# libAudioFlux/audioFlux

Hardware: AMD Instinct MI355X
Metric: audio frames/sec (mel+MFCC, n_fft=2048 hop=512) (higher is better)
Workload: dtype f32

## Files before the change

audioflux_amd/csrc/hip/afx_melfused2.hip:

```cpp
#include <hip/hip_runtime.h>

#include <cmath>
#include <cstdlib>
#include <cstring>

#include "afx_melplan.h"
#include "afx_melparts.h"
#include "afx_ccblock.h"

#ifdef AFX_V2_NTIN
#define AFX_V2_LOAD(p) __builtin_nontemporal_load(p)
#define AFX_V2_NT true
#else
#define AFX_V2_LOAD(p) (*(p))
#define AFX_V2_NT false
#endif
#ifndef AFX_V2_CCEVERY
#define AFX_V2_CCEVERY 16
#endif
#ifdef AFX_V2_STAMPS
#include <cstdio>
#include <vector>
#endif

namespace {

constexpr int NFFT = 2048;
constexpr int MC = 1024;
constexpr int WAVES = 12;
constexpr int WAVES_CPLX = 12;
__host__ __device__ constexpr int waves_of(bool cplx) { return cplx ? WAVES_CPLX : WAVES; }
constexpr int P1 = 72;
constexpr int PROW_OFF = 5120;
constexpr int PROW_F = 1104;
constexpr int WAVE_LDS = PROW_OFF + PROW_F * 4;
constexpr int CLAIM_LDS = 16;
static_assert(16 * P1 * 8 <= PROW_OFF + 1025 * 4, "exchange image must end before the zero pad");
constexpr int T_WIN = 0;
constexpr int T_TW1 = 8192;
constexpr int T_TW2 = 16384;
constexpr int TW2_PITCH = 144;
constexpr int T_TW3 = 16960;
constexpr int T_BAND = 21056;
__host__ __device__ constexpr int wpitch(int ta, int tb, int pc = 0) { return ta + tb + pc + 4; }
__host__ __device__ constexpr int tab_bytes(int ta, int tb, int pc = 0) { return T_BAND + 64 * wpitch(ta, tb, pc) * 4; }
constexpr int DCT_PITCH = 36;
__host__ __device__ constexpr int block_lds_bytes(int ta, int tb, bool cc, int pc = 0) {
    return tab_bytes(ta, tb, pc) + (cc ? 64 * DCT_PITCH * 4 : 0) + WAVES * WAVE_LDS + CLAIM_LDS;
}

__host__ __device__ constexpr int claim_length(int left, int waves, int minRun) {
    const int g = left / (2 * waves);
    if (left >= 16 * waves) return g >= 16 ? g & ~15 : 16;
    return (g & ~3) > minRun ? g & ~3 : minRun;
}

struct KArgs2 {
    const float *x;
    long long clipStride;
    long long totalFrames;
    int timeLength, hop;
    long long framesPerWg;
    int aligned;
    const float4 *tab;
    const int *meta;
    int specMap, postPow;
    float normValue;
    float *out;
    float *outIm;
    int num;
    const float *dct;
    int ccNum, ccCbrt;
    float *cc;
    float *energy, *rms, *zcr;
    const float *win;
    int binLo, binCount;
    long long outPitch;
    int vecOut;
#ifdef AFX_V2_STAMPS
    unsigned long long *stamps;
#endif
};
#ifdef AFX_V2_STAMPS
constexpr int STAMP_WORDS = 64, STAMP_HEAD = 8;
#endif


#ifndef AFX_PRIO_MASK
#define AFX_PRIO_MASK 0x1E
#endif
#ifndef AFX_PRIO_LEVEL
#define AFX_PRIO_LEVEL 1
#endif
#define MEL_PHASE(p)                                                                                       \
    do {                                                                                                   \
        if (AFX_PRIO_MASK != 0) __builtin_amdgcn_s_setprio(((AFX_PRIO_MASK >> (p)) & 1) ? AFX_PRIO_LEVEL : 0); \
    } while (0)

__device__ __forceinline__ float wave_sum(float v) {
#pragma unroll
    for (int o = 32; o > 0; o >>= 1) v += __shfl_xor(v, o, 64);
    return v;
}

template <int TA, int TB, int SHIFT, bool SPLIT, int CC, bool TEMPORAL, bool CPLX = false, bool STFT = false, int PC = 0>
__global__ __launch_bounds__(waves_of(CPLX) * 64, 3) void k_stft_mel_v2(KArgs2 a) {
    constexpr int NWV = waves_of(CPLX);
    static_assert(!(CPLX && (CC || TEMPORAL)), "complex results: the bank only");
    static_assert(!STFT || (TA == 0 && TB == 0 && !SPLIT && CC == 0 && !TEMPORAL && !CPLX), "STFT instantiations: real rows, no bank");
    static_assert(PC == 0 || (!SPLIT && !STFT), "packed plans hold whole rows");
    extern __shared__ __attribute__((aligned(16))) unsigned char smem[];
    const int lane = threadIdx.x & 63;
    const int wave = threadIdx.x >> 6;
    constexpr int WP = wpitch(TA, TB, PC);
    constexpr int TABB = tab_bytes(TA, TB, PC);
    constexpr int DCTB = CC == 1 ? 64 * DCT_PITCH * 4 : 0;
    unsigned char *wreg = smem + TABB + DCTB + wave * WAVE_LDS;
    float *prow = reinterpret_cast<float *>(wreg + PROW_OFF);

    {
        float4 *s4 = reinterpret_cast<float4 *>(smem);
        for (int i = threadIdx.x + (STFT ? T_TW1 / 16 : 0); i < TABB / 16; i += NWV * 64) s4[i] = a.tab[i];
        if constexpr (STFT) {
            v2 *tw = reinterpret_cast<v2 *>(smem + T_WIN);
            const v2 *w2 = reinterpret_cast<const v2 *>(a.win);
            for (int at = threadIdx.x; at < 1024; at += NWV * 64) {
                const int n1 = 2 * (at >> 7) + (at & 1), l = (at & 127) >> 1;
                tw[at] = w2[64 * n1 + l];
            }
        }
        if constexpr (CC == 1) {
            float *tabD = reinterpret_cast<float *>(smem + TABB);
            for (int i = threadIdx.x; i < 64 * 32; i += NWV * 64) {
                const int l = i >> 5, e = i & 31;
                const int fi = l & 15, g = l >> 4;
                tabD[l * DCT_PITCH + e] =
                    fi < a.ccNum ? a.dct[(long long)fi * a.num + 16 * (e >> 2) + 4 * g + (e & 3)] : 0.f;
            }
        }
        for (int i = 1025 + lane; i < PROW_F; i += 64) prow[i] = 0.f;
        if (threadIdx.x == 0) *reinterpret_cast<int *>(smem + TABB + DCTB + NWV * WAVE_LDS) = 0;
    }
    __syncthreads();

    const int k1 = lane >> 2, m2 = lane & 3;
    const unsigned T0 = lds_addr(smem), W0 = lds_addr(wreg);
    const unsigned aWin = T0 + T_WIN + 16 * lane;
    const unsigned aTw2 = T0 + T_TW2 + TW2_PITCH * m2;
    const unsigned aE1w = W0 + 8 * (8 * (k1 >> 1) + 2 * m2 + (k1 & 1));
    const unsigned aE1r = W0 + 576 * k1 + 16 * m2;
    const unsigned aE2w = W0 + 32 * k1 + 16 * ((m2 >> 1) ^ ((k1 >> 3) & 1)) + 8 * (m2 & 1);
    const int b3l = (lane >> 3) & 1;
    const unsigned aAlo = W0 + 32 * lane + 16 * b3l, aAhi = W0 + 32 * lane + 16 * (1 - b3l);
    const int qm0 = lane == 0 ? 128 : 256 - lane, qm1 = 192 - lane;
    const unsigned aB0lo = W0 + 32 * qm0 + 16 * ((qm0 >> 3) & 1), aB0hi = W0 + 32 * qm0 + 16 * (1 - ((qm0 >> 3) & 1));
    const unsigned aB1lo = W0 + 32 * qm1 + 16 * ((qm1 >> 3) & 1), aB1hi = W0 + 32 * qm1 + 16 * (1 - ((qm1 >> 3) & 1));
    const unsigned aT3lo = T0 + T_TW3 + 32 * lane + 16 * b3l, aT3hi = T0 + T_TW3 + 32 * lane + 16 * (1 - b3l);
    const unsigned R = W0 + PROW_OFF;
    const unsigned aP01 = R + 4 * lane;
    const unsigned aP23 = R + 4 * (lane == 0 ? 128 : lane + 512);
    const unsigned aQs1 = R + 4 * (192 - lane);
    const unsigned aQ23 = R + 4 * (lane == 0 ? 640 : 256 - lane);
    const bool lane0 = (lane == 0);

    constexpr int MROW = PC ? 192 : 128;
    const int startA = STFT ? 0 : a.meta[lane], startB = STFT ? 0 : a.meta[64 + lane], startC = PC ? a.meta[128 + lane] : 0;
    const int rowA = STFT ? -1 : a.meta[MROW + lane], rowB = STFT ? -1 : a.meta[MROW + 64 + lane], rowC = PC ? a.meta[MROW + 128 + lane] : -1;
    const unsigned seg0 = SPLIT ? (unsigned)a.meta[256 + lane] : 0u, seg1 = SPLIT ? (unsigned)a.meta[320 + lane] : 0u;
    const bool contB = PC ? a.meta[384 + lane] != 0 : false, contC = PC ? a.meta[448 + lane] != 0 : false;
    const unsigned apa = R + 4 * startA, apb = R + 4 * startB, apc = R + 4 * startC;
    const unsigned awr = T0 + T_BAND + 4 * WP * lane;
    const unsigned vRaw = 8u * (unsigned)lane, vLane = 4u * (unsigned)lane;
    const bool okA = rowA >= 0, okB = rowB >= 0, okC = rowC >= 0;
    const unsigned vRowA = okA ? 4u * (unsigned)rowA : 0u, vRowB = okB ? 4u * (unsigned)rowB : 0u, vRowC = okC ? 4u * (unsigned)rowC : 0u;
    const long long rowPitch = STFT ? a.outPitch : (long long)a.num;

    const long long wgBeg = (long long)blockIdx.x * a.framesPerWg;
    const int wgN = (int)(a.totalFrames - wgBeg < a.framesPerWg ? a.totalFrames - wgBeg : a.framesPerWg);
    const int minRun = wgN >= 4 * NWV ? 4 : wgN > NWV ? (wgN + NWV - 1) / NWV : 1;
    int *claimed = reinterpret_cast<int *>(smem + TABB + DCTB + NWV * WAVE_LDS);
    const int wgClip = (int)(wgBeg / a.timeLength);
    const unsigned wgT = (unsigned)(wgBeg - (long long)wgClip * a.timeLength);
    auto locate = [&](long long fr, int &c, int &tt) {
        const unsigned at = wgT + (unsigned)(fr - wgBeg);
        c = wgClip + (int)(at / (unsigned)a.timeLength);
        tt = (int)(at % (unsigned)a.timeLength);
    };
    auto claim = [&](long long &rb, long long &re) -> bool {
        int s = wgN, l = 0;
        if (lane0) {
            const int left = wgN - __atomic_load_n(claimed, __ATOMIC_RELAXED);
            if (left > 0) {
                l = claim_length(left, NWV, minRun);
                s = __atomic_fetch_add(claimed, l, __ATOMIC_RELAXED);
            }
        }
        s = __builtin_amdgcn_readfirstlane(s);
        l = __builtin_amdgcn_readfirstlane(l);
        if (s >= wgN) return false;
        rb = wgBeg + s;
        re = wgBeg + (s + l < wgN ? s + l : wgN);
        return true;
    };
    int ccN = 0;
#ifdef AFX_V2_STAMPS
    unsigned long long *stamp = a.stamps + ((long long)blockIdx.x * NWV + wave) * STAMP_WORDS;
    int stampN = 0;
    if (lane0) {
        stamp[0] = __builtin_amdgcn_s_memtime();
        stamp[2] = (unsigned long long)blockIdx.x | ((unsigned long long)wave << 32);
        stamp[4] = (unsigned)__builtin_amdgcn_s_getreg(4 | (0 << 6) | (31 << 11));
        stamp[5] = (unsigned)__builtin_amdgcn_s_getreg(20 | (0 << 6) | (31 << 11));
    }
#endif

    v2 raw[16];
    auto fetch = [&](const float *px, int first) {
        if (a.aligned) {
            const v2 *p2 = reinterpret_cast<const v2 *>(px);
#pragma unroll
            for (int n1 = 0; n1 < 16; ++n1)
                if (n1 >= first) raw[n1] = AFX_V2_LOAD(&p2[64 * n1 + lane]);
        } else {
#pragma unroll
            for (int n1 = 0; n1 < 16; ++n1)
                if (n1 >= first) {
                    const int n = 64 * n1 + lane;
                    raw[n1] = v2{px[2 * n], px[2 * n + 1]};
                }
        }
    };

    auto raw_landed = [&]() {
        if constexpr (SHIFT > 0) {
            VM_WAIT_ALL();
#pragma unroll
            for (int n1 = 0; n1 < 16; ++n1) PIN(raw[n1]);
        }
    };

    auto cc_block = [&](long long fb, long long fbS, int cnt) {
        if constexpr (CC == 2) {
            ccb_rows<SPLIT ? 2 : 4>(a.out, a.cc, a.dct, a.num, a.ccNum, a.ccCbrt, fb, cnt, lane);
        } else {
        VM_WAIT_ALL();
        int ln = lane;
        PIN(ln);
        const int fi = ln & 15, g = ln >> 4;
        fbS = uniform64(fbS);
        const float *const srows = a.out + fbS * 128;
        const unsigned vsrc = 512u * (unsigned)(fi < cnt ? fi : cnt - 1) + 16u * (unsigned)g;
        const unsigned ad = T0 + TABB + 4 * DCT_PITCH * ln;
        v4f acc[4] = {{0.f, 0.f, 0.f, 0.f}, {0.f, 0.f, 0.f, 0.f}, {0.f, 0.f, 0.f, 0.f}, {0.f, 0.f, 0.f, 0.f}};
        constexpr float LOG10_2 = 0.30102999566398120f;
#pragma unroll
        for (int h = 0; h < 2; ++h) {
            v4f av[4], dv[4];
            GLD128X4_L2_S(av[0], av[1], av[2], av[3], vsrc, srows, 256 * h, 256 * h + 64, 256 * h + 128, 256 * h + 192);
#pragma unroll
            for (int u = 0; u < 4; ++u) RD128(dv[u], ad, 16 * (4 * h + u));
            VM_LGKM_WAIT_ALL();
#pragma unroll
            for (int u = 0; u < 4; ++u) PIN(av[u]);
#pragma unroll
            for (int u = 0; u < 4; ++u) PIN(dv[u]);
#pragma unroll
            for (int u = 0; u < 4; ++u) {
                const v4f fl = max4_floor(av[u]);
#pragma unroll
                for (int c = 0; c < 4; ++c) {
                    const float lg = __log2f(fl[c]) * LOG10_2;
                    acc[c] = __builtin_amdgcn_mfma_f32_16x16x4f32(lg, dv[u][c], acc[c], 0, 0, 0);
                }
            }
        }
        const v4f sum = (acc[0] + acc[1]) + (acc[2] + acc[3]);
        if (fi < a.ccNum) {
            const unsigned vcc = 4u * (unsigned)(4 * g * a.ccNum + fi);
            float *const scc = a.cc + fbS * a.ccNum;
#pragma unroll
            for (int reg = 0; reg < 4; ++reg) {
                const int rr = 4 * g + reg;
                if (rr < cnt) GST32_S(vcc, sum[reg], scc + reg * a.ccNum);
            }
        }
        }
        ccN -= cnt;
    };

    long long fClaim, fEndClaim;
    while (claim(fClaim, fEndClaim)) {
    int laneZero = 0;
    PIN(laneZero);
    long long f = fClaim + laneZero;
    const long long fEnd = fEndClaim;
    int clip, t;
    locate(fClaim, clip, t);
    fetch(a.x + (long long)clip * a.clipStride + (long long)t * a.hop, 0);
    long long rowOff = fClaim * rowPitch;
    for (; f < fEnd; ++f) {
        v2 v[16];
        MEL_PHASE(0);
        {
            v4f wv[8];
#pragma unroll
            for (int j = 0; j < 8; ++j) RD128_S(2, wv[j], aWin, T_WIN + 1024 * j);
            LDS_WAIT_N(4);
#pragma unroll
            for (int j = 0; j < 4; ++j) {
                PIN(wv[j]);
                v[2 * j] = raw[2 * j] * lo2(wv[j]);
                v[2 * j + 1] = raw[2 * j + 1] * hi2(wv[j]);
            }
            LDS_WAIT_N(0);
#pragma unroll
            for (int j = 4; j < 8; ++j) {
                PIN(wv[j]);
                v[2 * j] = raw[2 * j] * lo2(wv[j]);
                v[2 * j + 1] = raw[2 * j + 1] * hi2(wv[j]);
            }
        }
        if constexpr (TEMPORAL) {
            float e = 0.f, z = 0.f;
            float prevTop = 0.f;
#pragma unroll
            for (int n1 = 0; n1 < 16; ++n1) {
                e = fmaf(v[n1].x, v[n1].x, e);
                e = fmaf(v[n1].y, v[n1].y, e);
                float py = __shfl_up(v[n1].y, 1, 64);
                if (lane0) py = prevTop;
                const bool first = (n1 == 0) && lane0;
                if (!first && v[n1].x * py < 0.f) z += 1.f;
                if (v[n1].y * v[n1].x < 0.f) z += 1.f;
                prevTop = __shfl(v[n1].y, 63, 64);
            }
            e = wave_sum(e);
            z = wave_sum(z);
            if (lane0) {
                a.energy[f] = e;
                a.rms[f] = sqrtf(e / (float)NFFT);
                a.zcr[f] = (float)((double)z / (double)NFFT);
            }
        }

        MEL_PHASE(1);
        dft16(v);
        {
            v4f tq[8];
#pragma unroll
            for (int j = 0; j < 8; ++j) RD128_S(2, tq[j], aWin, T_TW1 + 1024 * j);
            LDS_WAIT_N(0);
#pragma unroll
            for (int j = 0; j < 8; ++j) PIN(tq[j]);
            v2 o[16];
            o[0] = v[0];
#pragma unroll
            for (int k = 1; k < 16; ++k) o[k] = cmul(v[rev4(k)], (k & 1) ? hi2(tq[k >> 1]) : lo2(tq[k >> 1]));
#pragma unroll
            for (int g = 0; g < 4; ++g) {
                const unsigned b = aE1w + 2304 * g;
                WR2_64_S(0, b, o[4 * g], o[4 * g + 1], 0, 72);
                WR2_64_S(0, b, o[4 * g + 2], o[4 * g + 3], 144, 216);
            }
        }
        if (f + 1 < fEnd) {
            int tn = t + 1, cn = clip;
            if (tn == a.timeLength) {
                tn = 0;
                ++cn;
            }
            const float *pn = a.x + (long long)cn * a.clipStride + (long long)tn * a.hop;
            bool whole = true;
            if constexpr (SHIFT > 0) {
                if (tn != 0) {
                    shift_rows_inplace<SHIFT>(raw);
                    if (a.aligned) {
                        rows_fetch_new_s<SHIFT, AFX_V2_NT>(raw, vRaw, pn + 128 * (16 - SHIFT));
                    } else {
                        int z = 0;
                        VM_WAIT_ALL_AT(z);
                        fetch(pn + z, 16 - SHIFT);
                    }
                    whole = false;
                }
            }
            if (whole) {
                int z = 0;
                if constexpr (SHIFT > 0) VM_WAIT_ALL_AT(z);
                fetch(pn + z, 0);
            }
        }
        wave_lds_sync();
        MEL_PHASE(2);
        {
            v4f rq[8];
#pragma unroll
            for (int jj = 0; jj < 8; ++jj) RD128_S(1, rq[jj], aE1r, 64 * jj);
            wave_lds_sync();
#pragma unroll
            for (int jj = 0; jj < 8; ++jj) {
                PIN(rq[jj]);
                v[2 * jj] = lo2(rq[jj]);
                v[2 * jj + 1] = hi2(rq[jj]);
            }
        }

        MEL_PHASE(3);
        if (!KO_ON(5)) dft16(v);
        {
            v4f tq[8];
#pragma unroll
            for (int j = 0; j < 8; ++j) RD128_S(2, tq[j], aTw2, 16 * j);
            LDS_WAIT_N(0);
#pragma unroll
            for (int j = 0; j < 8; ++j) PIN(tq[j]);
            v2 o[16];
            o[0] = v[0];
#pragma unroll
            for (int j1 = 1; j1 < 16; ++j1) o[j1] = KO_ON(5) ? v[rev4(j1)] : cmul(v[rev4(j1)], (j1 & 1) ? hi2(tq[j1 >> 1]) : lo2(tq[j1 >> 1]));
#pragma unroll
            for (int g = 0; g < 4; ++g) {
                const unsigned b = aE2w + 2048 * g;
                WR2_64_S(0, b, o[4 * g], o[4 * g + 1], 0, 64);
                WR2_64_S(0, b, o[4 * g + 2], o[4 * g + 3], 128, 192);
            }
        }
        wave_lds_sync();

        MEL_PHASE(4);
        float pk[2][4], pq[2][4], p512;
        float ik[CPLX ? 2 : 1][4], iq[CPLX ? 2 : 1][4], i512 = 0.f;
        {
            v4f zalo[2], zahi[2], zblo[2], zbhi[2], wlo[2], whi[2];
            RD128_S(1, zalo[0], aAlo, 0);
            RD128_S(1, zahi[0], aAhi, 0);
            RD128_S(1, zblo[0], aB0lo, 0);
            RD128_S(1, zbhi[0], aB0hi, 0);
            RD128_S(2, wlo[0], aT3lo, 0);
            RD128_S(2, whi[0], aT3hi, 0);
            RD128_S(1, zalo[1], aAlo, 2048);
            RD128_S(1, zahi[1], aAhi, 2048);
            RD128_S(1, zblo[1], aB1lo, 0);
            RD128_S(1, zbhi[1], aB1hi, 0);
            RD128_S(2, wlo[1], aT3lo, 2048);
            RD128_S(2, whi[1], aT3hi, 2048);
#pragma unroll
            for (int s = 0; s < 2; ++s) {
                if (s == 0) LDS_WAIT_N(6);
                else LDS_WAIT_N(0);
                PIN(zalo[s]); PIN(zahi[s]); PIN(zblo[s]); PIN(zbhi[s]); PIN(wlo[s]); PIN(whi[s]);
                v2 za0 = lo2(zalo[s]), za1 = hi2(zalo[s]), za2 = lo2(zahi[s]), za3 = hi2(zahi[s]);
                v2 zb0 = lo2(zblo[s]), zb1 = hi2(zblo[s]), zb2 = lo2(zbhi[s]), zb3 = hi2(zbhi[s]);
                dft4(za0, za1, za2, za3);
                dft4(zb0, zb1, zb2, zb3);
                v2 A0 = za0, A1 = za1, A2 = za2, A3 = za3;
                v2 B0 = zb3, B1 = zb2, B2 = zb1, B3 = zb0;
                if (s == 0) {
                    if constexpr (CPLX) cplx_map(v2{za2.x, -za2.y}, a.specMap == 4, p512, i512);
                    else p512 = za2.x * za2.x + za2.y * za2.y;
                    A2 = lane0 ? zb0 : za2;
                    A3 = lane0 ? zb1 : za3;
                    B0 = lane0 ? za0 : zb3;
                    B1 = lane0 ? za3 : zb2;
                    B2 = lane0 ? zb3 : zb1;
                    B3 = lane0 ? zb2 : zb0;
                }
                if constexpr (CPLX) {
                    const bool sq = a.specMap == 4;
                    const v2 AA[4] = {A0, A1, A2, A3}, BB[4] = {B0, B1, B2, B3};
                    const v2 ww[4] = {lo2(wlo[s]), hi2(wlo[s]), lo2(whi[s]), hi2(whi[s])};
#pragma unroll
                    for (int j = 0; j < 4; ++j) {
                        v2 x, y;
                        split_pair_c(AA[j], BB[j], ww[j], x, y);
                        cplx_map(x, sq, pk[s][j], ik[CPLX ? s : 0][j]);
                        cplx_map(v2{y.x, -y.y}, sq, pq[s][j], iq[CPLX ? s : 0][j]);
                    }
                } else {
                    split_pair(A0, B0, lo2(wlo[s]), pk[s][0], pq[s][0]);
                    split_pair(A1, B1, hi2(wlo[s]), pk[s][1], pq[s][1]);
                    split_pair(A2, B2, lo2(whi[s]), pk[s][2], pq[s][2]);
                    split_pair(A3, B3, hi2(whi[s]), pk[s][3], pq[s][3]);
                }
            }
        }
        if constexpr (CPLX) {
            WR2ST_32(aP01 - PROW_OFF, ik[0][0], ik[0][1], 0, 4);
            WR2ST_32(aP23 - PROW_OFF, ik[0][2], ik[0][3], 0, 4);
            WR2ST_32(aP01 - PROW_OFF, ik[1][0], ik[1][1], 1, 5);
            WR2ST_32(aP01 - PROW_OFF, ik[1][2], ik[1][3], 9, 13);
            WR2ST_32(aQs1 - PROW_OFF, iq[0][1], iq[0][0], 9, 13);
            WR2ST_32(aQ23 - PROW_OFF, iq[0][3], iq[0][2], 0, 4);
            WR2ST_32(aQs1 - PROW_OFF, iq[1][3], iq[1][2], 0, 4);
            WR2ST_32(aQs1 - PROW_OFF, iq[1][1], iq[1][0], 8, 12);
            float *prowI = reinterpret_cast<float *>(wreg);
            if (lane0) prowI[512] = i512;
            prowI[1025 + lane] = 0.f;
            if (lane < PROW_F - 1025 - 64) prowI[1025 + 64 + lane] = 0.f;
        }
        WR2ST_32_S(4, aP01, pk[0][0], pk[0][1], 0, 4);
        WR2ST_32_S(4, aP23, pk[0][2], pk[0][3], 0, 4);
        WR2ST_32_S(4, aP01, pk[1][0], pk[1][1], 1, 5);
        WR2ST_32_S(4, aP01, pk[1][2], pk[1][3], 9, 13);
        WR2ST_32_S(4, aQs1, pq[0][1], pq[0][0], 9, 13);
        WR2ST_32_S(4, aQ23, pq[0][3], pq[0][2], 0, 4);
        WR2ST_32_S(4, aQs1, pq[1][3], pq[1][2], 0, 4);
        WR2ST_32_S(4, aQs1, pq[1][1], pq[1][0], 8, 12);
        if (lane0) prow[512] = p512;
        wave_lds_sync();
#pragma unroll
        for (int pass = 0; pass < (CPLX ? 2 : 1); ++pass) {
        const unsigned bpa = (CPLX && pass) ? apa - PROW_OFF : apa, bpb = (CPLX && pass) ? apb - PROW_OFF : apb;
        const unsigned bpc = (CPLX && pass) ? apc - PROW_OFF : apc;
        if (!CPLX && a.specMap) {
            for (int k = lane; k < 1025; k += 64) {
                const float p = prow[k];
                prow[k] = a.specMap == 1 ? sqrtf(p) : powf(p, a.normValue);
            }
            wave_lds_sync();
        }

        if constexpr (STFT) {
            MEL_PHASE(6);
            raw_landed();
            float *orow = a.out + rowOff;
            if (a.vecOut) {
                const float4 *p4 = reinterpret_cast<const float4 *>(prow);
                float4 *o4 = reinterpret_cast<float4 *>(orow);
                float4 q[4];
#pragma unroll
                for (int i = 0; i < 4; ++i) q[i] = p4[lane + 64 * i];
#pragma unroll
                for (int i = 0; i < 4; ++i) o4[lane + 64 * i] = q[i];
                if (lane0) o4[256] = p4[256];
            } else {
                for (int k = lane; k < a.binCount; k += 64) orow[k] = prow[a.binLo + k];
            }
        } else {
        MEL_PHASE(5);
        float accA, accB, accC = 0.f;
        if constexpr (PC > 0) {
            v2 sA, sB, sC;
            band_stage3<TA, TB, PC, 4, CPLX>(awr, bpa, bpb, bpc, contB, contC, sA, sB, sC);
            accA = sA.x + sA.y;
            accB = sB.x + sB.y;
            accC = sC.x + sC.y;
        } else {
            v2 sA, sB;
            band_stage<TA, TB, 4, CPLX>(awr, bpa, bpb, sA, sB);
            accA = sA.x + sA.y;
            accB = sB.x + sB.y;
        }
        if (!CPLX && !SPLIT && a.postPow) {
            accA = powf(accA, a.normValue);
            accB = powf(accB, a.normValue);
            if constexpr (PC > 0) accC = powf(accC, a.normValue);
        }
        MEL_PHASE(6);
        if (pass == 0) raw_landed();
        if constexpr (CC != 0 && !SPLIT) {
            if (ccN == AFX_V2_CCEVERY) cc_block(f - AFX_V2_CCEVERY, (rowOff >> 7) - AFX_V2_CCEVERY, AFX_V2_CCEVERY);
        }
        float *const srow = ((CPLX && pass) ? a.outIm : a.out) + rowOff;
        if constexpr (SPLIT) {
            float *part = reinterpret_cast<float *>(wreg + (CPLX ? PROW_F * 4 : 0));
            static_assert(PROW_F * 4 + 129 * 4 <= PROW_OFF, "segment sums must fit between the two rows");
            part[lane] = accA;
            part[64 + lane] = accB;
            if (lane0) part[128] = 0.f;
            wave_lds_sync();
#pragma unroll
            for (int h = 0; h < 2; ++h) {
                const unsigned u = h ? seg1 : seg0;
                float sum = part[u & 255u] + part[(u >> 8) & 255u];
                sum += part[(u >> 16) & 255u];
                sum += part[u >> 24];
                if (!CPLX && a.postPow) sum = powf(sum, a.normValue);
                if (lane + 64 * h < a.num) GST32_S(vLane, sum, srow + 64 * h);
            }
        } else {
            if (okA) GST32_S(vRowA, accA, srow);
            if (okB) GST32_S(vRowB, accB, srow);
            if constexpr (PC > 0) {
                if (okC) GST32_S(vRowC, accC, srow);
            }
        }
        if constexpr (CC != 0) {
            ++ccN;
            if (f + 1 == fEnd || (SPLIT && ccN == 16)) cc_block(f + 1 - ccN, (rowOff >> 7) + 1 - ccN, ccN);
        }
        }
        wave_lds_sync();

        }

#ifdef AFX_V2_STAMPS
        ++stampN;
        if (lane0 && (stampN & 15) == 0 && STAMP_HEAD + (stampN >> 4) <= STAMP_WORDS) stamp[STAMP_HEAD - 1 + (stampN >> 4)] = __builtin_amdgcn_s_memtime();
#endif
        rowOff += rowPitch;
        if (++t == a.timeLength) {
            t = 0;
            ++clip;
        }
    }
    }
#ifdef AFX_V2_STAMPS
    if (lane0) {
        stamp[1] = __builtin_amdgcn_s_memtime();
        stamp[3] = (unsigned long long)stampN;
    }
#endif
}

void fill_tables(float *tab, const float *hWindow) {
    const double PI = 3.14159265358979323846;
    float *win = tab + T_WIN / 4, *tw1 = tab + T_TW1 / 4, *tw2 = tab + T_TW2 / 4, *tw3 = tab + T_TW3 / 4;
    for (int n1 = 0; n1 < 16; ++n1)
        for (int l = 0; l < 64; ++l) {
            const int at = 2 * (128 * (n1 >> 1) + 2 * l + (n1 & 1));
            const int n = 64 * n1 + l;
            if (hWindow) {
                win[at] = hWindow[2 * n];
                win[at + 1] = hWindow[2 * n + 1];
            }
            const double ang = -2.0 * PI * (double)(n1 * l) / MC;
            tw1[at] = (float)cos(ang);
            tw1[at + 1] = (float)sin(ang);
        }
    for (int m = 0; m < 4; ++m)
        for (int j = 0; j < 16; ++j) {
            const double ang = -2.0 * PI * (double)(m * j) / 64.0;
            tw2[(TW2_PITCH / 4) * m + 2 * j] = (float)cos(ang);
            tw2[(TW2_PITCH / 4) * m + 2 * j + 1] = (float)sin(ang);
        }
    for (int s = 0; s < 2; ++s)
        for (int l = 0; l < 64; ++l)
            for (int m = 0; m < 4; ++m) {
                int bin = l + 64 * s + 256 * m;
                if (s == 0 && l == 0 && m >= 2) bin = m == 2 ? 128 : 384;
                const double ang = -2.0 * PI * (double)bin / NFFT;
                const int at = 2 * (4 * (64 * s + l) + 2 * ((m >> 1) ^ ((l >> 3) & 1)) + (m & 1));
                tw3[at] = (float)(0.5 * cos(ang));
                tw3[at + 1] = (float)(0.5 * sin(ang));
            }
}

constexpr AfxMelVariant kVariants[] = {{48, 16}, {72, 32}};

long long wg_ranges(long long total, int waves, long long *framesPerWg) {
    const char *e = getenv("AFX_MEL_CUS");
    const int asked = e ? atoi(e) : 0;
    const int cus = asked > 0 ? asked : afx_cu_count();
    long long fpw;
    long long blocks = afx_frame_split(total, cus, waves, 1, &fpw);
    *framesPerWg = fpw * waves;
    if (*framesPerWg > (1ll << 30)) {
        *framesPerWg = 1ll << 30;
        blocks = (total + *framesPerWg - 1) / *framesPerWg;
    }
    return blocks;
}

#ifdef AFX_V2_STAMPS
unsigned long long *stamps_begin(long long blocks, int waves) {
    unsigned long long *d = nullptr;
    const size_t n = (size_t)blocks * waves * STAMP_WORDS * 8;
    if (hipMalloc(&d, n) != hipSuccess || hipMemset(d, 0, n) != hipSuccess) return nullptr;
    return d;
}
void stamps_end(unsigned long long *d, long long blocks, int waves, void *stream) {
    const size_t n = (size_t)blocks * waves * STAMP_WORDS;
    std::vector<unsigned long long> h(n);
    (void)hipStreamSynchronize((hipStream_t)stream);
    if (hipMemcpy(h.data(), d, n * 8, hipMemcpyDeviceToHost) == hipSuccess)
        if (const char *name = getenv("AFX_V2_STAMPS_FILE"))
            if (FILE *fp = fopen(name, "wb")) {
                fwrite(h.data(), 8, n, fp);
                fclose(fp);
            }
    (void)hipFree(d);
}
#endif

template <int TA, int TB, int SHIFT, bool SPLIT, int CC, bool TEMPORAL, bool CPLX = false, int PC = 0>
int launch_variant(const AfxMelPlan *p, const AfxMelFusedArgs *a, void *stream) {
    const long long total = (long long)a->batch * a->timeLength;
    if (total <= 0) return AFX_OK;
    constexpr int NWV = waves_of(CPLX);
    long long fpg;
    const long long blocks = wg_ranges(total, NWV, &fpg);

    KArgs2 k;
    memset(&k, 0, sizeof(k));
    k.x = a->x;
    k.clipStride = a->clipStride;
    k.totalFrames = total;
    k.timeLength = a->timeLength;
    k.hop = a->hop;
    k.framesPerWg = fpg;
    k.aligned = ((a->clipStride & 1) == 0) && ((a->hop & 1) == 0) && ((reinterpret_cast<uintptr_t>(a->x) & 7) == 0);
    k.tab = reinterpret_cast<const float4 *>(p->dTab);
    k.meta = p->dMeta;
    k.specMap = a->specMap;
    k.postPow = a->postPow;
    k.normValue = a->normValue;
    k.out = a->out;
    k.outIm = a->outIm;
    k.num = p->num;
    k.dct = a->dct;
    k.ccNum = a->ccNum;
    k.ccCbrt = a->ccRectify == 1;
    k.cc = a->cc;
    k.energy = a->energy;
    k.rms = a->rms;
    k.zcr = a->zcr;
    constexpr size_t lds = (size_t)block_lds_bytes(TA, TB, CC == 1, PC);
    static_assert(lds <= 163840, "workgroup LDS budget");
#ifdef AFX_V2_STAMPS
    if (!(k.stamps = stamps_begin(blocks, NWV))) return AFX_ERR_HIP;
#endif
    AFX_LAUNCH_DYN_LDS((k_stft_mel_v2<TA, TB, SHIFT, SPLIT, CC, TEMPORAL, CPLX, false, PC>), dim3((unsigned)blocks), dim3(NWV * 64), lds, stream, k);
    AFX_LAUNCH_CHECK("k_stft_mel_v2");
#ifdef AFX_V2_STAMPS
    stamps_end(k.stamps, blocks, NWV, stream);
#endif
    return AFX_OK;
}

template <int TA, int TB, bool SPLIT, int CC, bool TEMPORAL, int PC = 0>
int launch_hop(const AfxMelPlan *p, const AfxMelFusedArgs *a, void *stream) {
#ifdef AFX_EXPERIMENTS
    if (const char *e = getenv("AFX_EXP_MEL"))
        if (strstr(e, "noshift")) return launch_variant<TA, TB, 0, SPLIT, CC, TEMPORAL, false, PC>(p, a, stream);
#endif
    switch (a->hop) {
        case 256: return launch_variant<TA, TB, 2, SPLIT, CC, TEMPORAL, false, PC>(p, a, stream);
        case 512: return launch_variant<TA, TB, 4, SPLIT, CC, TEMPORAL, false, PC>(p, a, stream);
        case 1024: return launch_variant<TA, TB, 8, SPLIT, CC, TEMPORAL, false, PC>(p, a, stream);
        default: return launch_variant<TA, TB, 0, SPLIT, CC, TEMPORAL, false, PC>(p, a, stream);
    }
}

template <int TA, int TB>
int launch(const AfxMelPlan *p, const AfxMelFusedArgs *a, void *stream) {
    const bool cc = a->cc != nullptr, tmp = a->energy != nullptr;
    if (a->specMap >= 3) {
        if (cc || tmp) return AFX_ERR_UNSUPPORTED;
        if (!a->outIm) return AFX_ERR_ARG;
        if (a->hop == 512)
            return p->split ? launch_variant<TA, TB, 4, true, 0, false, true>(p, a, stream)
                            : launch_variant<TA, TB, 4, false, 0, false, true>(p, a, stream);
        return p->split ? launch_variant<TA, TB, 0, true, 0, false, true>(p, a, stream)
                        : launch_variant<TA, TB, 0, false, 0, false, true>(p, a, stream);
    }
    if (cc && tmp) return AFX_ERR_UNSUPPORTED;
    if (cc) {
        if (a->ccNum < 1 || a->ccNum > 16 || !a->dct || !a->out || p->num > 128 || (p->num & 3)) return AFX_ERR_UNSUPPORTED;
        if (a->ccRectify != 0 && a->ccRectify != 1) return AFX_ERR_UNSUPPORTED;
        if constexpr (block_lds_bytes(TA, TB, true) <= 163840)
            if (!p->split && p->num == 128 && a->ccRectify == 0) return launch_hop<TA, TB, false, 1, false>(p, a, stream);
        if (a->hop == 512)
            return p->split ? launch_variant<TA, TB, 4, true, 2, false>(p, a, stream) : launch_variant<TA, TB, 4, false, 2, false>(p, a, stream);
        return p->split ? launch_variant<TA, TB, 0, true, 2, false>(p, a, stream) : launch_variant<TA, TB, 0, false, 2, false>(p, a, stream);
    }
    if (tmp) {
        if (!a->rms || !a->zcr) return AFX_ERR_ARG;
        return p->split ? launch_hop<TA, TB, true, 0, true>(p, a, stream)
                        : launch_hop<TA, TB, false, 0, true>(p, a, stream);
    }
    return p->split ? launch_hop<TA, TB, true, 0, false>(p, a, stream)
                    : launch_hop<TA, TB, false, 0, false>(p, a, stream);
}

template <int PA, int PB, int PC>
int launch_packed(const AfxMelPlan *p, const AfxMelFusedArgs *a, void *stream) {
    const bool cc = a->cc != nullptr, tmp = a->energy != nullptr;
    if (a->specMap >= 3) {
        if (cc || tmp) return AFX_ERR_UNSUPPORTED;
        if (!a->outIm) return AFX_ERR_ARG;
        if (a->hop == 512) return launch_variant<PA, PB, 4, false, 0, false, true, PC>(p, a, stream);
        return launch_variant<PA, PB, 0, false, 0, false, true, PC>(p, a, stream);
    }
    if (cc && tmp) return AFX_ERR_UNSUPPORTED;
    if (cc) {
        if (a->ccNum < 1 || a->ccNum > 16 || !a->dct || !a->out || p->num > 128 || (p->num & 3)) return AFX_ERR_UNSUPPORTED;
        if (a->ccRectify != 0 && a->ccRectify != 1) return AFX_ERR_UNSUPPORTED;
        static_assert(block_lds_bytes(PA, PB, true, PC) <= 163840, "the headline form: DCT operand in LDS");
        if (p->num == 128 && a->ccRectify == 0) return launch_hop<PA, PB, false, 1, false, PC>(p, a, stream);
        if (a->hop == 512) return launch_variant<PA, PB, 4, false, 2, false, false, PC>(p, a, stream);
        return launch_variant<PA, PB, 0, false, 2, false, false, PC>(p, a, stream);
    }
    if (tmp) {
        if (!a->rms || !a->zcr) return AFX_ERR_ARG;
        return launch_hop<PA, PB, false, 0, true, PC>(p, a, stream);
    }
    return launch_hop<PA, PB, false, 0, false, PC>(p, a, stream);
}

constexpr int kPacks[][3] = {{24, 12, 12}};

int run(const AfxMelPlan *p, const AfxMelFusedArgs *a, void *stream) {
    if (p->pack == 1) return launch_packed<24, 12, 12>(p, a, stream);
    return p->variant == 0 ? launch<48, 16>(p, a, stream) : launch<72, 32>(p, a, stream);
}

void fill_stft_tables(float *tab) { fill_tables(tab, nullptr); }

template <int SHIFT>
int launch_stft2k(const AfxStftArgs *a, const float *tab, void *stream) {
    const long long total = (long long)a->batch * a->timeLength;
    long long fpg;
    const long long blocks = wg_ranges(total, WAVES, &fpg);
    KArgs2 k;
    memset(&k, 0, sizeof(k));
    k.x = a->x;
    k.clipStride = a->clipStride;
    k.totalFrames = total;
    k.timeLength = a->timeLength;
    k.hop = a->hop;
    k.framesPerWg = fpg;
    k.aligned = ((a->clipStride & 1) == 0) && ((a->hop & 1) == 0) && ((reinterpret_cast<uintptr_t>(a->x) & 7) == 0);
    k.tab = reinterpret_cast<const float4 *>(tab);
    k.specMap = a->mode == AFX_SPEC_POWER ? 0 : a->mode == AFX_SPEC_MAG ? 1 : 2;
    k.normValue = a->normValue;
    k.out = a->outRe;
    k.win = a->window;
    k.binLo = a->binLo;
    k.binCount = a->binCount;
    k.outPitch = a->outPitch ? a->outPitch : (long long)a->binCount;
    k.vecOut = a->binLo == 0 && a->binCount == NFFT / 2 + 1 && k.outPitch >= 1028 && (k.outPitch & 3) == 0 &&
               (reinterpret_cast<uintptr_t>(a->outRe) & 15) == 0;
    constexpr size_t lds = (size_t)block_lds_bytes(0, 0, false);
#ifdef AFX_V2_STAMPS
    if (!(k.stamps = stamps_begin(blocks, WAVES))) return AFX_ERR_HIP;
#endif
    AFX_LAUNCH_DYN_LDS((k_stft_mel_v2<0, 0, SHIFT, false, 0, false, false, true>), dim3((unsigned)blocks), dim3(WAVES * 64), lds, stream, k);
    AFX_LAUNCH_CHECK("k_stft_mel_v2 (stft)");
#ifdef AFX_V2_STAMPS
    stamps_end(k.stamps, blocks, WAVES, stream);
#endif
    return AFX_OK;
}

}

const AfxMelSize *afx_mel_size2k() {
    static const AfxMelSize size = {11, 0, kVariants, 2, T_BAND, fill_tables, run, kPacks, 1, PROW_F};
    return &size;
}

extern "C" int afxk_stft2k(const AfxStftArgs *a, void *stream) {
    if (a->radix2Exp != 11 || a->bandStart || a->energy || a->padLeft != 0 || a->hop < 1 || a->binLo < 0 || a->binCount < 1 ||
        a->binLo + a->binCount > NFFT / 2 + 1 || (long long)(a->timeLength - 1) * a->hop + NFFT > a->dataLength ||
        (reinterpret_cast<uintptr_t>(a->window) & 7) != 0)
        return AFX_ERR_UNSUPPORTED;
    if (a->mode != AFX_SPEC_POWER && a->mode != AFX_SPEC_MAG && a->mode != AFX_SPEC_POWER_NORM) return AFX_ERR_UNSUPPORTED;
    if (!a->outRe) return AFX_ERR_ARG;
    const long long total = (long long)a->batch * a->timeLength;
    if (total <= 0) return AFX_OK;
    if (total > 0x7fffffffLL) return AFX_ERR_UNSUPPORTED;
    const float *tab = afx_device_table<fill_stft_tables>((size_t)tab_bytes(0, 0));
    if (!tab) return AFX_ERR_UNSUPPORTED;
    switch (a->hop) {
        case 256: return launch_stft2k<2>(a, tab, stream);
        case 512: return launch_stft2k<4>(a, tab, stream);
        case 1024: return launch_stft2k<8>(a, tab, stream);
        default: return launch_stft2k<0>(a, tab, stream);
    }
}
```

Before: 742.3 million.

## Fold W64 twiddle multiply into the radix-4 stage and relayout twiddle table

Moves the second-stage twiddle multiplication out of the phase-3 transpose write and into the phase-4 radix-4 butterfly. The W_64 table is relaid out as 16 compact rows of three twiddles indexed by the consumer's row. The reads are interleaved with the existing exchange loads, and the second-half tables can be loaded late to save registers. This removes a separate 8-read LDS wait and 15 complex multiplies before the exchange write, but adds 12 extra table reads per thread in the later stage. It also changes the priority mask to drop elevated priority for phase 3, and adds an exported host table-fill helper.

```diff
diff --git a/audioflux_amd/csrc/hip/afx_melfused2.hip b/audioflux_amd/csrc/hip/afx_melfused2.hip
--- a/audioflux_amd/csrc/hip/afx_melfused2.hip
+++ b/audioflux_amd/csrc/hip/afx_melfused2.hip
@@ -39,8 +39,9 @@
 constexpr int T_WIN = 0;
 constexpr int T_TW1 = 8192;
 constexpr int T_TW2 = 16384;
-constexpr int TW2_PITCH = 144;
+constexpr int TW2_PITCH = 32;
 constexpr int T_TW3 = 16960;
+static_assert(TW2_PITCH % 16 == 0 && T_TW2 + 16 * TW2_PITCH <= T_TW3, "W_64 table: 16-byte rows, ends before the split twiddles");
 constexpr int T_BAND = 21056;
 __host__ __device__ constexpr int wpitch(int ta, int tb, int pc = 0) { return ta + tb + pc + 4; }
 __host__ __device__ constexpr int tab_bytes(int ta, int tb, int pc = 0) { return T_BAND + 64 * wpitch(ta, tb, pc) * 4; }
@@ -87,7 +88,7 @@
 
 
 #ifndef AFX_PRIO_MASK
-#define AFX_PRIO_MASK 0x1E
+#define AFX_PRIO_MASK 0x16
 #endif
 #ifndef AFX_PRIO_LEVEL
 #define AFX_PRIO_LEVEL 1
@@ -146,7 +147,6 @@
     const int k1 = lane >> 2, m2 = lane & 3;
     const unsigned T0 = lds_addr(smem), W0 = lds_addr(wreg);
     const unsigned aWin = T0 + T_WIN + 16 * lane;
-    const unsigned aTw2 = T0 + T_TW2 + TW2_PITCH * m2;
     const unsigned aE1w = W0 + 8 * (8 * (k1 >> 1) + 2 * m2 + (k1 & 1));
     const unsigned aE1r = W0 + 576 * k1 + 16 * m2;
     const unsigned aE2w = W0 + 32 * k1 + 16 * ((m2 >> 1) ^ ((k1 >> 3) & 1)) + 8 * (m2 & 1);
@@ -155,6 +155,8 @@
     const int qm0 = lane == 0 ? 128 : 256 - lane, qm1 = 192 - lane;
     const unsigned aB0lo = W0 + 32 * qm0 + 16 * ((qm0 >> 3) & 1), aB0hi = W0 + 32 * qm0 + 16 * (1 - ((qm0 >> 3) & 1));
     const unsigned aB1lo = W0 + 32 * qm1 + 16 * ((qm1 >> 3) & 1), aB1hi = W0 + 32 * qm1 + 16 * (1 - ((qm1 >> 3) & 1));
+    const unsigned aTwA = T0 + T_TW2 + TW2_PITCH * (lane >> 4);
+    const unsigned aTwB0 = T0 + T_TW2 + TW2_PITCH * (qm0 >> 4), aTwB1 = T0 + T_TW2 + TW2_PITCH * (qm1 >> 4);
     const unsigned aT3lo = T0 + T_TW3 + 32 * lane + 16 * b3l, aT3hi = T0 + T_TW3 + 32 * lane + 16 * (1 - b3l);
     const unsigned R = W0 + PROW_OFF;
     const unsigned aP01 = R + 4 * lane;
@@ -408,16 +410,9 @@
         MEL_PHASE(3);
         if (!KO_ON(5)) dft16(v);
         {
-            v4f tq[8];
-#pragma unroll
-            for (int j = 0; j < 8; ++j) RD128_S(2, tq[j], aTw2, 16 * j);
-            LDS_WAIT_N(0);
-#pragma unroll
-            for (int j = 0; j < 8; ++j) PIN(tq[j]);
             v2 o[16];
-            o[0] = v[0];
-#pragma unroll
-            for (int j1 = 1; j1 < 16; ++j1) o[j1] = KO_ON(5) ? v[rev4(j1)] : cmul(v[rev4(j1)], (j1 & 1) ? hi2(tq[j1 >> 1]) : lo2(tq[j1 >> 1]));
+#pragma unroll
+            for (int j1 = 0; j1 < 16; ++j1) o[j1] = v[rev4(j1)];
 #pragma unroll
             for (int g = 0; g < 4; ++g) {
                 const unsigned b = aE2w + 2048 * g;
@@ -431,26 +426,58 @@
         float pk[2][4], pq[2][4], p512;
         float ik[CPLX ? 2 : 1][4], iq[CPLX ? 2 : 1][4], i512 = 0.f;
         {
-            v4f zalo[2], zahi[2], zblo[2], zbhi[2], wlo[2], whi[2];
+#ifdef AFX_V2_TABLATE
+            constexpr bool TAB_LATE = true;
+#else
+            constexpr bool TAB_LATE = STFT;
+#endif
+            v4f zalo[2], zahi[2], zblo[2], zbhi[2], wlo[2], whi[2], ta12[2], tb12[2];
+            v2 ta3[2], tb3[2];
+            auto tables_s1 = [&]() {
+                RD128_S(2, ta12[1], aTwA, 4 * TW2_PITCH);
+                RD64_S(2, ta3[1], aTwA, 4 * TW2_PITCH + 16);
+                RD128_S(2, tb12[1], aTwB1, 0);
+                RD64_S(2, tb3[1], aTwB1, 16);
+                RD128_S(2, wlo[1], aT3lo, 2048);
+                RD128_S(2, whi[1], aT3hi, 2048);
+            };
             RD128_S(1, zalo[0], aAlo, 0);
             RD128_S(1, zahi[0], aAhi, 0);
             RD128_S(1, zblo[0], aB0lo, 0);
             RD128_S(1, zbhi[0], aB0hi, 0);
+            RD128_S(2, ta12[0], aTwA, 0);
+            RD64_S(2, ta3[0], aTwA, 16);
+            RD128_S(2, tb12[0], aTwB0, 0);
+            RD64_S(2, tb3[0], aTwB0, 16);
             RD128_S(2, wlo[0], aT3lo, 0);
             RD128_S(2, whi[0], aT3hi, 0);
             RD128_S(1, zalo[1], aAlo, 2048);
             RD128_S(1, zahi[1], aAhi, 2048);
             RD128_S(1, zblo[1], aB1lo, 0);
             RD128_S(1, zbhi[1], aB1hi, 0);
-            RD128_S(2, wlo[1], aT3lo, 2048);
-            RD128_S(2, whi[1], aT3hi, 2048);
+            if constexpr (!TAB_LATE) tables_s1();
 #pragma unroll
             for (int s = 0; s < 2; ++s) {
-                if (s == 0) LDS_WAIT_N(6);
+                if (s == 0) LDS_WAIT_N(TAB_LATE ? 4 : 10);
                 else LDS_WAIT_N(0);
                 PIN(zalo[s]); PIN(zahi[s]); PIN(zblo[s]); PIN(zbhi[s]); PIN(wlo[s]); PIN(whi[s]);
+                PIN(ta12[s]); PIN(ta3[s]); PIN(tb12[s]); PIN(tb3[s]);
                 v2 za0 = lo2(zalo[s]), za1 = hi2(zalo[s]), za2 = lo2(zahi[s]), za3 = hi2(zahi[s]);
                 v2 zb0 = lo2(zblo[s]), zb1 = hi2(zblo[s]), zb2 = lo2(zbhi[s]), zb3 = hi2(zbhi[s]);
+                if (!KO_ON(5)) {
+                    za1 = cmul(za1, lo2(ta12[s]));
+                    za2 = cmul(za2, hi2(ta12[s]));
+                    za3 = cmul(za3, ta3[s]);
+                    zb1 = cmul(zb1, lo2(tb12[s]));
+                    zb2 = cmul(zb2, hi2(tb12[s]));
+                    zb3 = cmul(zb3, tb3[s]);
+                }
+                if constexpr (TAB_LATE) {
+                    if (s == 0) {
+                        PIN(za1); PIN(za2); PIN(za3); PIN(zb1); PIN(zb2); PIN(zb3);
+                        tables_s1();
+                    }
+                }
                 dft4(za0, za1, za2, za3);
                 dft4(zb0, zb1, zb2, zb3);
                 v2 A0 = za0, A1 = za1, A2 = za2, A3 = za3;
@@ -628,12 +655,14 @@
             tw1[at] = (float)cos(ang);
             tw1[at + 1] = (float)sin(ang);
         }
-    for (int m = 0; m < 4; ++m)
-        for (int j = 0; j < 16; ++j) {
+    for (int j = 0; j < 16; ++j) {
+        for (int m = 1; m < 4; ++m) {
             const double ang = -2.0 * PI * (double)(m * j) / 64.0;
-            tw2[(TW2_PITCH / 4) * m + 2 * j] = (float)cos(ang);
-            tw2[(TW2_PITCH / 4) * m + 2 * j + 1] = (float)sin(ang);
-        }
+            tw2[(TW2_PITCH / 4) * j + 2 * (m - 1)] = (float)cos(ang);
+            tw2[(TW2_PITCH / 4) * j + 2 * (m - 1) + 1] = (float)sin(ang);
+        }
+        tw2[(TW2_PITCH / 4) * j + 6] = tw2[(TW2_PITCH / 4) * j + 7] = 0.f;
+    }
     for (int s = 0; s < 2; ++s)
         for (int l = 0; l < 64; ++l)
             for (int m = 0; m < 4; ++m) {
@@ -850,6 +879,14 @@
     return &size;
 }
 
+extern "C" int afxk_mel2k_tables(float *tab, int bytes) {
+    if (tab && bytes >= T_BAND) {
+        memset(tab, 0, T_BAND);
+        fill_tables(tab, nullptr);
+    }
+    return T_BAND;
+}
+
 extern "C" int afxk_stft2k(const AfxStftArgs *a, void *stream) {
     if (a->radix2Exp != 11 || a->bandStart || a->energy || a->padLeft != 0 || a->hop < 1 || a->binLo < 0 || a->binCount < 1 ||
         a->binLo + a->binCount > NFFT / 2 + 1 || (long long)(a->timeLength - 1) * a->hop + NFFT > a->dataLength ||
```

After: 754.8 million (median of 6 runs). 1.02x the previous value.
